# ericzzj1989/BALF

Measured on AMD Instinct MI355X. Metric: images/sec + keypoints/sec on 1080p gray (detector forward + NMS + top-K); NMS index match vs CPU ref, higher is better.
Workload: dtype f16 MFMA, split hi+lo operands (3 products), f32 accumulate/LN/GELU/softmax/NMS

## Files before the change

balf_amd/_lib.py:

```python
from __future__ import annotations

import ctypes as C
import os

_HERE = os.path.dirname(os.path.abspath(__file__))
LIB_PATH = os.environ.get("BALF_HIP_LIB", os.path.join(_HERE, "libbalf_hip.so"))

OK = 0
PREC_FP32, PREC_FP16 = 0, 1
MAX_NMS_SIZE, MAX_TOPK = 32, 16384
PYR_SRC_U8, PYR_SRC_F32, PYR_SRC_LEVEL = 0, 1, 2
PYR_MAX_RADIUS, MAX_PYRAMID_LEVELS = 8, 32
VAL_LEG_GREEDY, VAL_LEG_WINDOW = 0, 1
STATUS_SCORE, STATUS_RANGE, STATUS_SE, STATUS_WORDS = 0, 1, 2, 4

_vp, _i, _sz, _fp = C.c_void_p, C.c_int, C.c_size_t, C.c_void_p
PROTOTYPES = {
    "balf_abi_version": (_i, []),
    "balf_error_string": (C.c_char_p, [_i]),
    "balf_device_check": (_i, []),
    "balf_build_flags": (C.c_char_p, []),
    "balf_num_state_tensors": (_i, []),
    "balf_state_tensor_name": (C.c_char_p, [_i]),
    "balf_state_tensor_numel": (_sz, [_i]),
    "balf_packed_weights_bytes": (_sz, [_i]),
    "balf_pack_weights": (_i, [C.POINTER(_vp), _i, _i, _vp, _sz]),
    "balf_forward_workspace_bytes": (_sz, [_i, _i, _i]),
    "balf_forward_micro_batch": (_i, [_i, _i, _i]),
    "balf_forward": (_i, [_vp, _i, _fp, _i, _i, _i, _fp, _fp, _vp, _sz, _vp]),
    "balf_forward_u8": (_i, [_vp, _i, _vp, _i, _i, _i, _i, _fp, _fp, _vp, _sz, _vp]),
    "balf_forward_status": (_i, [_vp, _i, _fp, _i, _i, _i, _fp, _fp, _vp, _sz, _vp, _vp]),
    "balf_forward_u8_status": (_i, [_vp, _i, _vp, _i, _i, _i, _i, _fp, _fp, _vp, _sz, _vp, _vp]),
    "balf_forward_stage_view_numel": (_sz, [_i, _i, _i, _i]),
    "balf_forward_stage_view": (_i, [_i, _vp, _sz, _i, _i, _i, _i, _fp, _vp]),
    "balf_window_nms": (_i, [_fp, _i, _i, _i, _i, _i, _fp, _vp]),
    "balf_nms_topk_workspace_bytes": (_sz, [_i, _i, _i, _i]),
    "balf_nms_topk": (_i, [_fp, _i, _i, _i, _i, _i, _i, _i, _i, _i, _i, _vp, _fp, _vp, _vp, _sz, _vp]),
    "balf_nms_threshold": (_i, [_fp, _i, _i, _i, _i, _i, _i, _i, _i, _i, C.c_float, _i, _vp, _fp, _vp, _vp, _sz, _vp]),
    "balf_pyramid_level": (_i, [_vp, _i, _i, _i, _i, _i, C.c_double, _i, _i, _fp, _vp]),
    "balf_nms_topk_budget": (_i, [_fp, _i, _i, _i, _i, _i, _i, _i, _i, _i, _i, _i, _vp, _vp, _fp, _vp, _vp, _sz, _vp]),
    "balf_multiscale_merge": (_i, [_vp, _fp, _vp, _i, _i, _i, _vp, _vp, _i, _i, _vp, _vp, _vp]),
    "balf_greedy_nms_workspace_bytes": (_sz, [_i, _i, _i, _i]),
    "balf_greedy_nms": (_i, [_fp, _i, _i, _i, _i, _i, _i, _i, _i, C.c_float, _i, _i, _i, _vp, _fp, _fp, _vp, _vp, _vp,
                            _sz, _vp]),
    "balf_hardnet_num_state_tensors": (_i, []),
    "balf_hardnet_state_tensor_name": (C.c_char_p, [_i]),
    "balf_hardnet_state_tensor_numel": (_sz, [_i]),
    "balf_hardnet_packed_weights_bytes": (_sz, []),
    "balf_hardnet_pack_weights": (_i, [C.POINTER(_vp), _i, _vp, _sz]),
    "balf_hardnet_workspace_bytes": (_sz, [_i]),
    "balf_hardnet_forward": (_i, [_vp, _fp, _i, _fp, _vp, _sz, _vp]),
    "balf_hardnet_forward_masked": (_i, [_vp, _fp, _i, _i, _vp, _fp, _vp, _sz, _vp]),
    "balf_hardnet_forward_ex": (_i, [_vp, _fp, _i, _i, _vp, _i, _fp, _vp, _sz, _vp]),
    "balf_extract_patches_workspace_bytes": (_sz, [_i, _i, C.c_float]),
    "balf_extract_patches": (_i, [_vp, _i, _i, _fp, _i, C.c_float, _fp, _vp, _sz, _vp]),
    "balf_extract_patches_batch_workspace_bytes": (_sz, [_i, _i, _i, C.c_float]),
    "balf_extract_patches_batch": (_i, [_vp, _i, _i, _i, _fp, _vp, _i, C.c_float, _fp, _vp, _sz, _vp]),
    "balf_rgb_to_gray": (_i, [_vp, C.c_long, _vp, _vp]),
    "balf_match_smnn_workspace_bytes": (_sz, [_i, _i]),
    "balf_match_smnn": (_i, [_fp, _i, _fp, _i, C.c_float, _vp, _fp, _vp, _vp, _sz, _vp]),
    "balf_match_smnn_batch_workspace_bytes": (_sz, [_i, _i, _i]),
    "balf_match_smnn_batch": (_i, [_fp, _i, _vp, _fp, _i, _vp, _i, C.c_float, _vp, _fp, _vp, _vp, _sz, _vp]),
    "balf_repeatability_workspace_bytes": (_sz, [_i, _i, _i]),
    "balf_repeatability": (_i, [_vp, _i, _vp, _i, C.c_double, C.c_double, C.c_double, C.c_double, _i, _vp, _vp, _vp, _vp,
                               _vp, _sz, _vp]),
    "balf_apply_homography": (_i, [_vp, _i, _vp, _vp, _vp]),
    "balf_common_region_masks": (_i, [_vp, _i, _i, _i, _i, _i, _vp, _vp, _vp]),
    "balf_common_points_batch": (_i, [_vp, _vp, _i, _vp, _vp, _i, _i, _vp, _vp, _vp, _vp, _vp, _vp, _vp]),
    "balf_repeatability_batch_workspace_bytes": (_sz, [_i, _i, _i, _i]),
    "balf_repeatability_batch": (_i, [_vp, _vp, _i, _i, _vp, _vp, _i, _i, _i, _i, C.c_double, C.c_double, C.c_double,
                                     C.c_double, _i, _vp, _vp, _vp, _sz, _vp]),
    "balf_common_points_index_batch": (_i, [_vp, _vp, _i, _vp, _vp, _i, _i, _vp, _vp, _vp, _vp, _vp, _vp, _vp, _vp, _vp]),
    "balf_match_accuracy_batch": (_i, [_vp, _i, _vp, _i, _vp, _vp, _vp, _i, _i, C.POINTER(C.c_double), _i, _vp, _vp, _vp]),
    "balf_val_points_workspace_bytes": (_sz, [_i, _i, _i, _i, _i, _i, _i, _i]),
    "balf_val_points": (_i, [_fp, _i, _i, _fp, _i, _i, _i, _vp, _i, C.c_float, _i, _i, _vp, _vp, _vp, _vp, _sz, _vp]),
    "balf_resize_repeatability_batch_workspace_bytes": (_sz, [_i, _i, _i, _i]),
    "balf_resize_repeatability_batch": (_i, [_vp, _vp, _i, _i, _vp, _vp, _i, _i, _i, _i, _i, _vp, _vp, _vp, _i, C.c_double,
                                            _vp, _vp, _vp, _sz, _vp]),
    "balf_resize_crop_u8": (_i, [_vp, _sz, _vp, _vp, _i, _i, _i, _i, _vp, _vp]),
    "balf_synth_pairs_workspace_bytes": (_sz, [_i, _i]),
    "balf_synth_pairs": (_i, [_vp, _sz, _vp, _vp, _i, _vp, _vp, _vp, _fp, _i, _vp, _i, _i, _fp, _fp, _fp, _fp, _vp, _vp, _sz,
                             _vp]),
    "balf_detector_loss_workspace_bytes": (_sz, [_i, _i, _i]),
    "balf_detector_loss": (_i, [_fp, _fp, _fp, _fp, _i, _i, _i, _fp, _fp, _vp, _fp, _vp, _sz, _vp]),
    "balf_head_train_workspace_bytes": (_sz, [C.c_long]),
    "balf_head_train_saved_bytes": (_sz, [C.c_long]),
    "balf_head_train_forward": (_i, [_fp, _fp, _fp, _fp, _fp, _fp, _fp, _i, _i, _i, C.c_double, _i, _fp, _fp, _fp, _fp, _fp,
                                    C.c_double, _vp, _vp, _sz, _vp]),
    "balf_head_train_backward": (_i, [_fp, _fp, _fp, _fp, _fp, _vp, _i, _i, _i, _fp, _fp, _fp, _fp, _fp, _fp, _fp, _vp, _sz, _vp]),
    "balf_rcab_train_workspace_bytes": (_sz, [_i, _i, _i]),
    "balf_rcab_train_saved_bytes": (_sz, [_i, _i, _i]),
# ... 102 lines not shown
```

balf_amd/csrc/nms_topk.hip:

```cpp
#include <cstdint>
#include <cstdlib>
#include "block_ops.h"
#include "common.h"
#include "prof.h"

namespace {

constexpr int TH = 64;
constexpr int TW = 64;
constexpr int SEG = 16;
constexpr int NTHREADS = 256;

template <int SIZE, int N>
__device__ __forceinline__ void window_max_1d(const float (&v)[N + SIZE - 1], float (&o)[N]) {
    if constexpr (SIZE == 15) {
        constexpr int L = N + 14;
        float a[L - 1], b[L - 3], c[L - 7];
#pragma unroll
        for (int i = 0; i < L - 1; ++i) a[i] = fmaxf(v[i], v[i + 1]);
#pragma unroll
        for (int i = 0; i < L - 3; ++i) b[i] = fmaxf(a[i], a[i + 2]);
#pragma unroll
        for (int i = 0; i < L - 7; ++i) c[i] = fmaxf(b[i], b[i + 4]);
#pragma unroll
        for (int i = 0; i < N; ++i) o[i] = fmaxf(c[i], c[i + 7]);
    } else {
#pragma unroll
        for (int i = 0; i < N; ++i) {
            float m = v[i];
#pragma unroll
            for (int k = 1; k < SIZE; ++k) m = fmaxf(m, v[i + k]);
            o[i] = m;
        }
    }
}

struct NmsArgs {
    const float *src;
    int Hs, Ws;
    int crop_y, crop_x;
    int H, W;
    int border;
    int size;
    int2 *surv;
    int *surv_count;
    long cap;
    float *dense;
};

__device__ __forceinline__ float load_score(const NmsArgs &a, const float *img, int y, int x) {
    if (y < 0 || y >= a.H || x < 0 || x >= a.W) return -INFINITY;
    if (y < a.border || y >= a.H - a.border || x < a.border || x >= a.W - a.border) return 0.0f;
    return img[(long)(a.crop_y + y) * a.Ws + (a.crop_x + x)];
// ... 237 lines not shown
    const int b = blockIdx.z;
    const int ty0 = blockIdx.y * TH, tx0 = blockIdx.x * TW;
    const float *img = a.src + (long)b * a.Hs * a.Ws;
    const int tid = threadIdx.x;

    for (int i = tid; i < IN_H * IN_W; i += NTHREADS) {
        const int r = i / IN_W, c = i - r * IN_W;
        s_in[r * PIN + c] = load_score(a, img, ty0 - LO + r, tx0 - LO + c);
    }
    __syncthreads();
    for (int i = tid; i < IN_H * TW; i += NTHREADS) {
        const int r = i / TW, c = i - r * TW;
        float m = s_in[r * PIN + c];
        for (int k = 1; k < size; ++k) m = fmaxf(m, s_in[r * PIN + c + k]);
        s_row[r * PROW + c] = m;
    }
    __syncthreads();

    const int x = tid & (TW - 1), seg = tid / TW;
    const int gx = tx0 + x;
    unsigned keepmask = 0;
    float cen[SEG];
    for (int j = 0; j < SEG; ++j) {
        const int ry = seg * SEG + j;
        float m = s_row[ry * PROW + x];
        for (int k = 1; k < size; ++k) m = fmaxf(m, s_row[(ry + k) * PROW + x]);
        const int gy = ty0 + ry;
        cen[j] = s_in[(ry + LO) * PIN + x + LO];
        const bool inside = (gy < a.H) && (gx < a.W);
        const bool keep = inside && (cen[j] == m);
        if (a.dense != nullptr) {
            if (inside) a.dense[((long)b * a.H + gy) * a.W + gx] = cen[j] * (keep ? 1.0f : 0.0f);
        } else if (keep && cen[j] > 0.0f) {
            keepmask |= 1u << j;
        }
    }
    if (a.dense != nullptr) return;

    int total;
    const int excl = block_exclusive_scan(__popc(keepmask), s_scan, &total);
    if (total == 0) return;
    if (tid == 0) s_base = atomicAdd(&a.surv_count[b], total);
    __syncthreads();
    long pos = (long)b * a.cap + s_base + excl;
    for (int j = 0; j < SEG; ++j) {
        if (keepmask & (1u << j)) {
            const int gy = ty0 + seg * SEG + j;
            a.surv[pos++] = make_int2(gy * a.W + gx, __float_as_int(cen[j]));
        }
    }
}

constexpr int SEL_THREADS = 1024;

__global__ __launch_bounds__(SEL_THREADS) void topk_select_kernel(const int2 *surv_all, const int *surv_count,
                                                                  long cap, int K, int npow2, int zero_fallback,
                                                                  unsigned thr_explicit, int32_t *idx_out,
                                                                  float *score_out, int32_t *count_out,
                                                                  int32_t *taken, int cum_budget) {
    extern __shared__ __attribute__((aligned(16))) unsigned char smem[];
    unsigned long long *keys = reinterpret_cast<unsigned long long *>(smem);
    unsigned *s_hist = reinterpret_cast<unsigned *>(keys + npow2);
    int *s_tmp = reinterpret_cast<int *>(s_hist + 256);
    int *s_cnt = s_tmp + 4;

    const int b = blockIdx.x;
    const int2 *surv = surv_all + (long)b * cap;
    const int n = surv_count[b];
    const int K_row = K;
    int32_t *idx_o = idx_out + (long)b * K_row;
    float *sc_o = score_out + (long)b * K_row;
    if (taken) {
        if (threadIdx.x == 0) {
            long kb = (long)cum_budget - taken[b];
            kb = kb < cap ? kb : cap;
            kb = kb < K_row ? kb : K_row;
            *s_cnt = kb > 0 ? (int)kb : 0;
        }
        __syncthreads();
        K = *s_cnt;
        __syncthreads();
        npow2 = balf::next_pow2(K);
    }

    if (K == 0 || (n == 0 && (!zero_fallback || thr_explicit))) {
        for (int i = threadIdx.x; i < K_row; i += SEL_THREADS) { idx_o[i] = -1; sc_o[i] = 0.0f; }
        if (threadIdx.x == 0) count_out[b] = 0;
        return;
    }
    if (n == 0) {
        for (int i = threadIdx.x; i < K_row; i += SEL_THREADS) { idx_o[i] = i < K ? i : -1; sc_o[i] = 0.0f; }
        if (threadIdx.x == 0) {
            count_out[b] = K;
            if (taken) taken[b] += K;
        }
        return;
    }

    constexpr int CACHE = 16;
    const bool cached = n <= CACHE * SEL_THREADS;
    int2 ent[CACHE];
    if (cached) {
#pragma unroll
        for (int j = 0; j < CACHE; ++j) {
            const int i = threadIdx.x + j * SEL_THREADS;
            ent[j] = (i < n) ? surv[i] : make_int2(0x7fffffff, 0);
        }
    }
    const int n_mine = (n - (int)threadIdx.x + SEL_THREADS - 1) / SEL_THREADS;
    auto each = [&](auto f) {
        if (cached) {
#pragma unroll
            for (int j = 0; j < CACHE; ++j)
                if (j < n_mine) f(ent[j]);
        } else {
            for (int i = threadIdx.x; i < n; i += SEL_THREADS) f(surv[i]);
        }
    };

    unsigned thr = 0;
    int idx_cut = 0x7fffffff;
    auto raster_cut = [&]() {
        int d0, d1;
        const unsigned t = thr;
        return (int)balf::radix_select<32, false, SEL_THREADS>(
            K, [&](auto count) { each([&](int2 e) { if ((unsigned)e.y >= t) count((unsigned)e.x); }); }, s_hist, s_tmp, &d0, &d1);
    };
    if (thr_explicit) {
        thr = thr_explicit;
        if (threadIdx.x == 0) *s_cnt = 0;
        __syncthreads();
        int mine = 0;
        each([&](int2 e) { if ((unsigned)e.y >= thr) ++mine; });
        if (mine) atomicAdd(s_cnt, mine);
        __syncthreads();
        const int reach = *s_cnt;
        __syncthreads();
        if (reach > K) idx_cut = raster_cut();
    } else if (n > K) {
        int n_eq, need_eq;
        thr = (unsigned)balf::radix_select<32, true, SEL_THREADS>(
            K, [&](auto count) { each([&](int2 e) { count((unsigned)e.y); }); }, s_hist, s_tmp, &n_eq, &need_eq);
        if (n_eq > need_eq) idx_cut = raster_cut();
    }

    if (threadIdx.x == 0) *s_cnt = 0;
    for (int i = threadIdx.x; i < npow2; i += SEL_THREADS) keys[i] = ~0ull;
    __syncthreads();
    each([&](int2 e) {
        const unsigned sb = (unsigned)e.y;
        if (sb >= thr && e.x <= idx_cut) {
            const int p = atomicAdd(s_cnt, 1);
            keys[p] = ((unsigned long long)(~sb) << 32) | (unsigned)e.x;
        }
    });
    __syncthreads();
    const int cnt = *s_cnt;

    balf::bitonic_sort<SEL_THREADS>(keys, npow2);
    for (int i = threadIdx.x; i < K_row; i += SEL_THREADS) {
        if (i < cnt) {
            const unsigned long long kv = keys[i];
            idx_o[i] = (int32_t)(unsigned)(kv & 0xffffffffull);
            sc_o[i] = __uint_as_float(~(unsigned)(kv >> 32));
        } else {
            idx_o[i] = -1;
            sc_o[i] = 0.0f;
        }
    }
    if (threadIdx.x == 0) {
        count_out[b] = cnt;
        if (taken) taken[b] += cnt;
    }
}

int launch_nms_tiles(const NmsArgs &a, int B, hipStream_t stream) {
    dim3 grid(balf_ceil_div(a.W, TW), balf_ceil_div(a.H, TH), B), block(NTHREADS);
    if (balf_prof::g_on) balf_prof::before(balf_prof::kNmsTile, stream);
    static const bool no_vec = getenv("BALF_NMS_NO_VEC") != nullptr;
    if (a.size == 15 && a.dense == nullptr && !no_vec && a.Ws % 4 == 0 && a.crop_x % 4 == 0 &&
        (reinterpret_cast<uintptr_t>(a.src) & 15) == 0 && ((long)a.Hs * a.Ws) % 4 == 0) {
        hipLaunchKernelGGL(nms_tile15_vec_kernel, dim3(balf_ceil_div(a.W, TW), balf_ceil_div(a.H, V_TH), B), block, 0, stream, a);
        if (balf_prof::g_on) balf_prof::after(stream);
        BALF_LAUNCH_CHECK();
        return BALF_OK;
    }
    switch (a.size) {
        case 15: hipLaunchKernelGGL(nms_tile_kernel<15>, grid, block, 0, stream, a); break;
        case 5: hipLaunchKernelGGL(nms_tile_kernel<5>, grid, block, 0, stream, a); break;
        case 3: hipLaunchKernelGGL(nms_tile_kernel<3>, grid, block, 0, stream, a); break;
        default: hipLaunchKernelGGL(nms_tile_kernel_generic, grid, block, 0, stream, a); break;
    }
    if (balf_prof::g_on) balf_prof::after(stream);
    BALF_LAUNCH_CHECK();
    return BALF_OK;
}

}

namespace {
__global__ __launch_bounds__(256) void fill_u32_kernel(unsigned *dst, unsigned value, size_t n) {
    for (size_t i = (size_t)blockIdx.x * 256 + threadIdx.x; i < n; i += (size_t)gridDim.x * 256) dst[i] = value;
}
}

int balf_fill_u32(void *dst_dev, unsigned value, size_t n_words, hipStream_t stream) {
    if (n_words == 0) return BALF_OK;
    const size_t blocks = (n_words + 255) / 256;
    hipLaunchKernelGGL(fill_u32_kernel, dim3((unsigned)(blocks < 1024 ? blocks : 1024)), dim3(256), 0, stream,
                       static_cast<unsigned *>(dst_dev), value, n_words);
    BALF_LAUNCH_CHECK();
    return BALF_OK;
}

int balf_topk_select_launch(const int2 *surv, const int *counts, long cap, int B, int K, int zero_fallback,
                            int32_t *idx_dev, float *score_dev, int32_t *count_dev, hipStream_t st,
                            unsigned thr_explicit, int32_t *taken_dev, int cum_budget) {
    const int npow2 = balf::next_pow2(K);
    const size_t smem = (size_t)npow2 * 8 + 256 * 4 + 8 * 4;
    if (smem > 48 * 1024 &&
        hipFuncSetAttribute(reinterpret_cast<const void *>(topk_select_kernel),
                            hipFuncAttributeMaxDynamicSharedMemorySize, (int)smem) != hipSuccess)
        return BALF_ERR_LAUNCH;
    BALF_PROF(balf_prof::kTopkSelect, st,
              hipLaunchKernelGGL(topk_select_kernel, dim3(B), dim3(SEL_THREADS), smem, st, surv, counts, cap, K, npow2,
                                 zero_fallback, thr_explicit, idx_dev, score_dev, count_dev, taken_dev, cum_budget));
    BALF_LAUNCH_CHECK();
    return BALF_OK;
}

extern "C" int balf_window_nms(const float *score_dev, int B, int H, int W, int border, int nms_size,
                               float *out_dev, void *stream) {
    if (!score_dev || !out_dev || B <= 0 || H <= 0 || W <= 0 || border < 0) return BALF_ERR_ARG;
    if (nms_size < 1 || nms_size > BALF_MAX_NMS_SIZE) return BALF_ERR_ARG;
    if ((long)H * W > 0x7fffffffL) return BALF_ERR_SHAPE;
    NmsArgs a{score_dev, H, W, 0, 0, H, W, border, nms_size, nullptr, nullptr, 0, out_dev};
    return launch_nms_tiles(a, B, (hipStream_t)stream);
}

extern "C" size_t balf_nms_topk_workspace_bytes(int B, int H, int W, int K) {
    if (B <= 0 || H <= 0 || W <= 0 || K <= 0) return 0;
    return balf_align_up((size_t)B * sizeof(int), 256) + (size_t)B * (size_t)H * (size_t)W * sizeof(int2);
}

namespace {
int nms_select(const float *prob_dev, int B, int Hp, int Wp, int crop_y, int crop_x, int H, int W, int border,
               int nms_size, int K, unsigned thr_explicit, int32_t *idx_dev, float *score_dev, int32_t *count_dev,
               void *workspace_dev, size_t workspace_bytes, void *stream, int32_t *taken_dev = nullptr,
               int cum_budget = 0) {
    if (!prob_dev || !idx_dev || !score_dev || !count_dev || !workspace_dev) return BALF_ERR_ARG;
    if (B <= 0 || H <= 0 || W <= 0 || K <= 0 || border < 0) return BALF_ERR_ARG;
    if (nms_size < 1 || nms_size > BALF_MAX_NMS_SIZE || K > BALF_MAX_TOPK) return BALF_ERR_ARG;
    if (crop_y < 0 || crop_x < 0 || crop_y + H > Hp || crop_x + W > Wp) return BALF_ERR_SHAPE;
    if ((long)H * W > 0x7fffffffL || (!taken_dev && (long)K > (long)H * W)) return BALF_ERR_SHAPE;
    if (workspace_bytes < balf_nms_topk_workspace_bytes(B, H, W, K)) return BALF_ERR_WORKSPACE;
    hipStream_t st = (hipStream_t)stream;

    int *counts = reinterpret_cast<int *>(workspace_dev);
    int2 *surv = reinterpret_cast<int2 *>(reinterpret_cast<char *>(workspace_dev) +
                                          balf_align_up((size_t)B * sizeof(int), 256));
    if (balf_fill_u32(counts, 0u, balf_align_up((size_t)B * sizeof(int), 256) / 4, st) != BALF_OK) return BALF_ERR_LAUNCH;
    NmsArgs a{prob_dev, Hp, Wp, crop_y, crop_x, H, W, border, nms_size, surv, counts, (long)H * W, nullptr};
    int rc = launch_nms_tiles(a, B, st);
    if (rc != BALF_OK) return rc;

    return balf_topk_select_launch(surv, counts, (long)H * W, B, K, 1, idx_dev, score_dev, count_dev, st,
                                   thr_explicit, taken_dev, cum_budget);
}
}

int balf_window_survivors_launch(const float *prob_dev, int B, int H, int W, int nms_size, int2 *surv, int *counts,
                                 hipStream_t st) {
    if (balf_fill_u32(counts, 0u, (size_t)B, st) != BALF_OK) return BALF_ERR_LAUNCH;
    NmsArgs a{prob_dev, H, W, 0, 0, H, W, 0, nms_size, surv, counts, (long)H * W, nullptr};
    return launch_nms_tiles(a, B, st);
}

extern "C" int balf_nms_topk(const float *prob_dev, int B, int Hp, int Wp, int crop_y, int crop_x, int H, int W,
                             int border, int nms_size, int K, int32_t *idx_dev, float *score_dev,
                             int32_t *count_dev, void *workspace_dev, size_t workspace_bytes, void *stream) {
    return nms_select(prob_dev, B, Hp, Wp, crop_y, crop_x, H, W, border, nms_size, K, 0u, idx_dev, score_dev, count_dev,
                      workspace_dev, workspace_bytes, stream);
}

extern "C" int balf_nms_threshold(const float *prob_dev, int B, int Hp, int Wp, int crop_y, int crop_x, int H, int W,
                                  int border, int nms_size, float threshold, int K, int32_t *idx_dev, float *score_dev,
                                  int32_t *count_dev, void *workspace_dev, size_t workspace_bytes, void *stream) {
    if (!(threshold > 0.0f) || !(threshold < INFINITY)) return BALF_ERR_ARG;
    const unsigned bits = __builtin_bit_cast(unsigned, threshold);
    return nms_select(prob_dev, B, Hp, Wp, crop_y, crop_x, H, W, border, nms_size, K, bits, idx_dev, score_dev, count_dev,
                      workspace_dev, workspace_bytes, stream);
}

extern "C" int balf_nms_topk_budget(const float *prob_dev, int B, int Hp, int Wp, int crop_y, int crop_x, int H, int W,
                                    int border, int nms_size, int cum_budget, int K_max, int32_t *taken_dev,
                                    int32_t *idx_dev, float *score_dev, int32_t *count_dev, void *workspace_dev,
                                    size_t workspace_bytes, void *stream) {
    if (!taken_dev || cum_budget < 0 || cum_budget > K_max) return BALF_ERR_ARG;
    return nms_select(prob_dev, B, Hp, Wp, crop_y, crop_x, H, W, border, nms_size, K_max, 0u, idx_dev, score_dev, count_dev,
                      workspace_dev, workspace_bytes, stream, taken_dev, cum_budget);
}
```

balf_amd/ops.py:

```python
from __future__ import annotations

import ctypes as C
from typing import Dict, NamedTuple, Optional, Tuple

import numpy as np
import torch

from . import _lib
from .arch import padded_hw
from ._lib import BalfHipError, check, current_stream_ptr, lib, require_gpu_tensor

_workspaces: Dict[Tuple[str, int, int], torch.Tensor] = {}
_MAX_STREAMS_PER_TAG = 2


def _workspace(tag: str, device, nbytes: int) -> torch.Tensor:
    dev_index = device.index if device.index is not None else torch.cuda.current_device()
    key = (tag, dev_index, torch.cuda.current_stream(device).cuda_stream)
    ws = _workspaces.pop(key, None)
    if ws is None or ws.numel() < nbytes:
        ws = None
        with torch.cuda.device(device):
            ws = torch.empty(max(nbytes, 256), dtype=torch.uint8, device=device)
        same = [k for k in _workspaces if k[0] == tag and k[1] == dev_index]
        for k in same[:max(0, len(same) - (_MAX_STREAMS_PER_TAG - 1))]:
            del _workspaces[k]
    _workspaces[key] = ws
    return ws


def release_workspaces() -> None:
    _workspaces.clear()


def window_nms(score: torch.Tensor, border: int, nms_size: int) -> torch.Tensor:
    require_gpu_tensor(score, "score")
    if score.dtype != torch.float32 or score.dim() != 3:
        raise BalfHipError("score must be a [B,H,W] float32 tensor")
    out = torch.empty_like(score)
    b, h, w = score.shape
    with torch.cuda.device(score.device):
        check(lib().balf_window_nms(score.data_ptr(), b, h, w, int(border), int(nms_size), out.data_ptr(),
                                    current_stream_ptr(score.device)), "balf_window_nms")
    return out


def nms_topk(prob: torch.Tensor, crop_y: int, crop_x: int, h: int, w: int, border: int, nms_size: int,
             k: int, threshold: float = -1.0) -> Tuple[torch.Tensor, torch.Tensor, torch.Tensor]:
    require_gpu_tensor(prob, "prob")
    if prob.dtype != torch.float32 or prob.dim() != 3:
        raise BalfHipError("prob must be a [B,Hp,Wp] float32 tensor")
    if k > h * w:
        raise IndexError(f"index {k - 1} is out of bounds for axis 0 with size {h * w}")
    b, hp, wp = prob.shape
    dev = prob.device
    idx = torch.empty((b, k), dtype=torch.int32, device=dev)
    score = torch.empty((b, k), dtype=torch.float32, device=dev)
    count = torch.empty((b,), dtype=torch.int32, device=dev)
    nbytes = lib().balf_nms_topk_workspace_bytes(b, h, w, k)
    ws = _workspace("nms", dev, nbytes)
    with torch.cuda.device(dev):
        if threshold == -1:
            check(lib().balf_nms_topk(prob.data_ptr(), b, hp, wp, int(crop_y), int(crop_x), int(h), int(w),
                                      int(border), int(nms_size), int(k), idx.data_ptr(), score.data_ptr(),
                                      count.data_ptr(), ws.data_ptr(), ws.numel(), current_stream_ptr(dev)),
                  "balf_nms_topk")
        else:
            check(lib().balf_nms_threshold(prob.data_ptr(), b, hp, wp, int(crop_y), int(crop_x), int(h), int(w),
                                           int(border), int(nms_size), float(threshold), int(k), idx.data_ptr(),
                                           score.data_ptr(), count.data_ptr(), ws.data_ptr(), ws.numel(),
                                           current_stream_ptr(dev)), "balf_nms_threshold")
    return idx, score, count


def greedy_nms(prob: torch.Tensor, crop_y: int, crop_x: int, h: int, w: int, border: int, conf_thresh: float,
               dist_thresh: int, k: int, subpixel_patch: int = 0):
    require_gpu_tensor(prob, "prob")
    if prob.dtype != torch.float32 or prob.dim() != 3:
        raise BalfHipError("prob must be a [B,Hp,Wp] float32 tensor")
    b, hp, wp = prob.shape
    dev = prob.device
    idx = torch.empty((b, k), dtype=torch.int32, device=dev)
    score = torch.empty((b, k), dtype=torch.float32, device=dev)
    xy = torch.empty((b, k, 2), dtype=torch.float32, device=dev) if subpixel_patch > 0 else None
    count = torch.empty((b,), dtype=torch.int32, device=dev)
    total = torch.empty((b,), dtype=torch.int32, device=dev)
    ws = _workspace("greedy", dev, lib().balf_greedy_nms_workspace_bytes(b, h, w, k))
    with torch.cuda.device(dev):
        check(lib().balf_greedy_nms(prob.data_ptr(), b, hp, wp, int(crop_y), int(crop_x), int(h), int(w), int(border),
                                    float(conf_thresh), int(dist_thresh), int(k), int(subpixel_patch), idx.data_ptr(),
                                    score.data_ptr(), xy.data_ptr() if xy is not None else None, count.data_ptr(),
                                    total.data_ptr(), ws.data_ptr(), ws.numel(), current_stream_ptr(dev)),
              "balf_greedy_nms")
    return idx, score, xy, count, total


def profile_begin() -> None:
    check(lib().balf_profile_begin(), "balf_profile_begin")


def profile_end():
    l = lib()
    n = l.balf_profile_num_slots()
    ms = (C.c_float * n)()
    cnt = (C.c_int * n)()
    check(l.balf_profile_end(ms, cnt), "balf_profile_end")
    return {l.balf_profile_slot_name(i).decode(): (float(ms[i]), int(cnt[i])) for i in range(n) if cnt[i]}


def extract_patches(gray_u8: torch.Tensor, xy: torch.Tensor, scale: float) -> torch.Tensor:
    require_gpu_tensor(gray_u8, "gray_u8")
    if not xy.is_cuda:
        raise BalfHipError("xy must live on the GPU")
    if gray_u8.dtype != torch.uint8 or gray_u8.dim() != 2:
        raise BalfHipError("gray_u8 must be a [H,W] uint8 tensor")
    if xy.dim() != 2 or xy.shape[1] != 2:
        raise BalfHipError("xy must be [N,2]")
    xy = xy.contiguous().float()
    n = xy.shape[0]
    h, w = gray_u8.shape
    dev = gray_u8.device
    out = torch.empty((n, 1, 32, 32), dtype=torch.float32, device=dev)
    if n == 0:
        return out
    nbytes = lib().balf_extract_patches_workspace_bytes(h, w, float(scale))
# ... 729 lines not shown
```

balf_amd/pipeline.py:

```python
from __future__ import annotations

from typing import Optional, Tuple

import numpy as np
import torch

from . import arch, ops
from .guard import run_guarded
from .utils import test_utils as T


def detect_batch(model, x_pad: torch.Tensor, h: int, w: int, border: int = 15, nms_size: int = 15,
                 num_points: int = 1000, precomputed_offsets: Optional[Tuple[int, int]] = None, want_logits: bool = False):
    hp, wp = x_pad.shape[-2:]
    if precomputed_offsets is None:
        ehp, ewp, top, left = arch.padded_hw(h, w)
        if (ehp, ewp) != (hp, wp):
            raise ValueError(f"a {h}x{w} image pads to {ehp}x{ewp}, got {hp}x{wp}")
    else:
        top, left = precomputed_offsets
    prob = model(x_pad, want_logits=want_logits)["prob"]
    idx, score, count = ops.nms_topk(prob, top, left, h, w, border, nms_size, num_points)
    return idx, score, count, prob

# ... 62 lines not shown

@torch.no_grad()
def extract_detections(image_RGB_norm, model, device, cell_size=8, nms_size=15, num_points=25, border_size=15):
    h, w = image_RGB_norm.shape[0], image_RGB_norm.shape[1]
    x = pad_image_on_device(image_RGB_norm, device)

    def run():
        idx, score, count, prob = detect_batch(model, x, h, w, border_size, nms_size, num_points)
        return idx, score, int(count[0]), prob
    idx, score, n, prob = run_guarded(model, run)
    i = idx[0, :n].cpu().numpy().astype(np.int64)
    pts = np.empty((n, 4), dtype=np.float64)
    pts[:, 0], pts[:, 1], pts[:, 2], pts[:, 3] = i % w, i // w, 1.0, score[0, :n].cpu().numpy()
    _, _, top, left = arch.padded_hw(h, w)
    return pts, prob[:, top:top + h, left:left + w].unsqueeze(1)


def shard_range(total: int, rank: int, world: int) -> Tuple[int, int]:
    base, extra = divmod(total, world)
    lo = rank * base + min(rank, extra)
    return lo, lo + base + (1 if rank < extra else 0)


_SHAPES_CHECKED = set()


def allgather_keypoints(idx: torch.Tensor, score: torch.Tensor, count: torch.Tensor, group=None, force: bool = False,
                        total: Optional[int] = None):
    import torch.distributed as dist
    if not (dist.is_available() and dist.is_initialized()):
        return idx, score, count
    if dist.get_world_size(group) == 1 and not force:
        return idx, score, count
    world, rank = dist.get_world_size(group), dist.get_rank(group)
    b, k = idx.shape
    if total is None:
        rows = b
        key = (id(group) if group is not None else 0, world, b, k, str(idx.device))
        if key not in _SHAPES_CHECKED:
            mine = torch.tensor([b, k], dtype=torch.int64, device=idx.device)
            seen = torch.empty(world * 2, dtype=torch.int64, device=idx.device)
            dist.all_gather_into_tensor(seen, mine, group=group)
            seen = seen.view(world, 2)
            if not bool((seen == mine).all()):
                raise ValueError(f"allgather_keypoints: slab shapes differ across ranks ({seen.tolist()}); pass total= for the "
                                 f"unequal shards of shard_range")
            _SHAPES_CHECKED.add(key)
        shard_rows = [b] * world
    else:
        rows = -(-total // world)
        shard_rows = [shard_range(total, r, world)[1] - shard_range(total, r, world)[0] for r in range(world)]
        if shard_rows[rank] != b:
            raise ValueError(f"allgather_keypoints: rank {rank} of {world} holds {b} images, shard_range({total}) gives {shard_rows[rank]}")
    slab = torch.empty((rows, 2 * k + 1), dtype=torch.int32, device=idx.device)
    slab[:b, :k] = idx
    slab[:b, k:2 * k] = score.view(torch.int32)
    slab[:b, 2 * k] = count
    if rows > b:
        slab[b:, :k] = -1
        slab[b:, k:] = 0
    out = torch.empty((world * rows, 2 * k + 1), dtype=torch.int32, device=idx.device)
    dist.all_gather_into_tensor(out, slab, group=group)
    if any(r != rows for r in shard_rows):
        keep = torch.cat([torch.arange(r * rows, r * rows + shard_rows[r], device=idx.device) for r in range(world)])
        out = out.index_select(0, keep)
    return out[:, :k].contiguous(), out[:, k:2 * k].contiguous().view(torch.float32), out[:, 2 * k].contiguous()
```

include/balf_hip.h:

```cpp
#ifndef BALF_HIP_H
#define BALF_HIP_H

#include <stddef.h>
#include <stdint.h>

#ifdef __cplusplus
extern "C" {
#endif

#define BALF_ABI_VERSION 1

#define BALF_OK 0
#define BALF_ERR_ARG (-1)
#define BALF_ERR_SHAPE (-2)
#define BALF_ERR_WORKSPACE (-3)
#define BALF_ERR_ARCH (-4)
#define BALF_ERR_LAUNCH (-5)

#define BALF_MAX_NMS_SIZE 32
#define BALF_MAX_TOPK 16384

#define BALF_PREC_FP32 0
#define BALF_PREC_FP16 1

int balf_abi_version(void);
const char *balf_error_string(int code);
int balf_device_check(void);
const char *balf_build_flags(void);

int balf_num_state_tensors(void);
const char *balf_state_tensor_name(int i);
size_t balf_state_tensor_numel(int i);
size_t balf_packed_weights_bytes(int precision);
int balf_pack_weights(const float *const *tensors, int n_tensors, int precision,
                      void *packed_host, size_t packed_bytes);

size_t balf_forward_workspace_bytes(int B, int Hp, int Wp);
int balf_forward_micro_batch(int B, int Hp, int Wp);
int balf_forward(const void *packed_dev, int precision, const float *x_nchw_dev, int B, int Hp, int Wp,
                 float *logits_dev, float *prob_dev, void *workspace_dev, size_t workspace_bytes,
                 void *stream);

int balf_forward_u8(const void *packed_dev, int precision, const unsigned char *image_dev, int channels, int B,
                    int H, int W, float *logits_dev, float *prob_dev, void *workspace_dev, size_t workspace_bytes,
                    void *stream);

#define BALF_STATUS_SCORE 0
#define BALF_STATUS_RANGE 1
#define BALF_STATUS_SE 2
#define BALF_STATUS_WORDS 4
int balf_forward_status(const void *packed_dev, int precision, const float *x_nchw_dev, int B, int Hp, int Wp,
                        float *logits_dev, float *prob_dev, void *workspace_dev, size_t workspace_bytes,
                        int *status_dev, void *stream);
int balf_forward_u8_status(const void *packed_dev, int precision, const unsigned char *image_dev, int channels, int B,
                           int H, int W, float *logits_dev, float *prob_dev, void *workspace_dev, size_t workspace_bytes,
                           int *status_dev, void *stream);

size_t balf_forward_stage_view_numel(int B, int Hp, int Wp, int stage);
int balf_forward_stage_view(int precision, const void *workspace_dev, size_t workspace_bytes, int B, int Hp, int Wp, int stage,
                            float *out_dev, void *stream);

int balf_window_nms(const float *score_dev, int B, int H, int W, int border, int nms_size,
                    float *out_dev, void *stream);

size_t balf_nms_topk_workspace_bytes(int B, int H, int W, int K);
int balf_nms_topk(const float *prob_dev, int B, int Hp, int Wp, int crop_y, int crop_x, int H, int W,
                  int border, int nms_size, int K, int32_t *idx_dev, float *score_dev,
                  int32_t *count_dev, void *workspace_dev, size_t workspace_bytes, void *stream);

int balf_nms_threshold(const float *prob_dev, int B, int Hp, int Wp, int crop_y, int crop_x, int H, int W,
                       int border, int nms_size, float threshold, int K, int32_t *idx_dev, float *score_dev,
                       int32_t *count_dev, void *workspace_dev, size_t workspace_bytes, void *stream);

#define BALF_PYR_SRC_U8 0
#define BALF_PYR_SRC_F32 1
#define BALF_PYR_SRC_LEVEL 2
#define BALF_PYR_MAX_RADIUS 8
#define BALF_MAX_PYRAMID_LEVELS 32
int balf_pyramid_level(const void *src_dev, int src_kind, int channels, int B, int H_in, int W_in, double sigma, int H_out,
                       int W_out, float *dst_dev, void *stream);

int balf_nms_topk_budget(const float *prob_dev, int B, int Hp, int Wp, int crop_y, int crop_x, int H, int W, int border,
                         int nms_size, int cum_budget, int K_max, int32_t *taken_dev, int32_t *idx_dev, float *score_dev,
                         int32_t *count_dev, void *workspace_dev, size_t workspace_bytes, void *stream);

int balf_multiscale_merge(const int32_t *idx_dev, const float *score_dev, const int32_t *count_dev, int L, int B, int K_max,
                          const int32_t *level_w_host, const double *h_host, int N, int order_yx, double *pts_dev,
                          int32_t *count_out_dev, void *stream);

size_t balf_greedy_nms_workspace_bytes(int B, int H, int W, int K);
int balf_greedy_nms(const float *prob_dev, int B, int Hp, int Wp, int crop_y, int crop_x, int H, int W, int border,
                    float conf_thresh, int dist_thresh, int K, int subpixel_patch, int32_t *idx_dev,
                    float *score_dev, float *xy_dev, int32_t *count_dev, int32_t *total_dev, void *workspace_dev,
                    size_t workspace_bytes, void *stream);

int balf_hardnet_num_state_tensors(void);
const char *balf_hardnet_state_tensor_name(int i);
size_t balf_hardnet_state_tensor_numel(int i);
size_t balf_hardnet_packed_weights_bytes(void);
int balf_hardnet_pack_weights(const float *const *tensors, int n_tensors, void *packed_host, size_t packed_bytes);
size_t balf_hardnet_workspace_bytes(int n_patches);
int balf_hardnet_forward(const void *packed_dev, const float *patches_dev, int n_patches, float *desc_dev,
                         void *workspace_dev, size_t workspace_bytes, void *stream);
int balf_hardnet_forward_masked(const void *packed_dev, const float *patches_dev, int n_patches, int group,
                                const int32_t *count_dev, float *desc_dev, void *workspace_dev, size_t workspace_bytes,
                                void *stream);
#define BALF_HARDNET_SPLIT_F16 0
#define BALF_HARDNET_PLAIN_F16 1
int balf_hardnet_forward_ex(const void *packed_dev, const float *patches_dev, int n_patches, int group,
                            const int32_t *count_dev, int precision, float *desc_dev, void *workspace_dev,
                            size_t workspace_bytes, void *stream);

size_t balf_extract_patches_workspace_bytes(int H, int W, float scale);
int balf_extract_patches(const unsigned char *gray_dev, int H, int W, const float *xy_dev, int n_points, float scale,
                         float *patches_dev, void *workspace_dev, size_t workspace_bytes, void *stream);
size_t balf_extract_patches_batch_workspace_bytes(int B, int H, int W, float scale);
int balf_extract_patches_batch(const unsigned char *gray_dev, int B, int H, int W, const float *xy_dev,
                               const int32_t *count_dev, int K, float scale, float *patches_dev, void *workspace_dev,
                               size_t workspace_bytes, void *stream);
int balf_rgb_to_gray(const unsigned char *rgb_dev, long n_pixels, unsigned char *gray_dev, void *stream);
size_t balf_match_smnn_workspace_bytes(int n1, int n2);
size_t balf_match_smnn_batch_workspace_bytes(int pairs, int k1, int k2);
int balf_match_smnn_batch(const float *desc1_dev, int k1, const int32_t *n1_dev, const float *desc2_dev, int k2,
                          const int32_t *n2_dev, int pairs, float th, int32_t *idx_dev, float *dist_dev,
                          int32_t *count_dev, void *workspace_dev, size_t workspace_bytes, void *stream);
// ... 112 lines not shown
```

Baseline: 913.9.

## Split top-K select across CUs with global histogram, wave-level sort and output slab

Top-K selection now launches several blocks per image. Each block builds a 12-bit score histogram over a slice of the survivors and accumulates it into a global histogram, and the last block to arrive picks the threshold bin and runs a narrower radix select inside that bin. It also adds ballot-based compaction of the selected keys, a bitonic sort that does its small strides with wave shuffles, and a packed idx/score/count slab output so that all-gather can skip a repack copy. The aim is to use more CUs than images and to cut sort and compaction overhead, at the cost of extra workspace, global atomics and a last-block-done pattern that relies on relaxed ordering.

New measurement: 914.1, median of 6. About the same (+0.0%).

```diff
diff --git a/balf_amd/_lib.py b/balf_amd/_lib.py
--- a/balf_amd/_lib.py
+++ b/balf_amd/_lib.py
@@ -37,6 +37,7 @@
     "balf_nms_topk_workspace_bytes": (_sz, [_i, _i, _i, _i]),
     "balf_nms_topk": (_i, [_fp, _i, _i, _i, _i, _i, _i, _i, _i, _i, _i, _vp, _fp, _vp, _vp, _sz, _vp]),
     "balf_nms_threshold": (_i, [_fp, _i, _i, _i, _i, _i, _i, _i, _i, _i, C.c_float, _i, _vp, _fp, _vp, _vp, _sz, _vp]),
+    "balf_nms_topk_slab": (_i, [_fp, _i, _i, _i, _i, _i, _i, _i, _i, _i, C.c_float, _i, _vp, _vp, _sz, _vp]),
     "balf_pyramid_level": (_i, [_vp, _i, _i, _i, _i, _i, C.c_double, _i, _i, _fp, _vp]),
     "balf_nms_topk_budget": (_i, [_fp, _i, _i, _i, _i, _i, _i, _i, _i, _i, _i, _i, _vp, _vp, _fp, _vp, _vp, _sz, _vp]),
     "balf_multiscale_merge": (_i, [_vp, _fp, _vp, _i, _i, _i, _vp, _vp, _i, _i, _vp, _vp, _vp]),
diff --git a/balf_amd/csrc/nms_topk.hip b/balf_amd/csrc/nms_topk.hip
--- a/balf_amd/csrc/nms_topk.hip
+++ b/balf_amd/csrc/nms_topk.hip
@@ -1,4 +1,5 @@
 #include <cstdint>
+#include <atomic>
 #include <cstdlib>
 #include "block_ops.h"
 #include "common.h"
@@ -342,24 +343,88 @@
 }
 
 constexpr int SEL_THREADS = 1024;
+constexpr int SLICE_BITS = 12, SLICE_BINS = 1 << SLICE_BITS, SLICE_SHIFT = 31 - SLICE_BITS;
+constexpr int MAX_SLICES = 16;
+__device__ __forceinline__ unsigned slice_bin(unsigned score_bits) { return (score_bits >> SLICE_SHIFT) & (unsigned)(SLICE_BINS - 1); }
+
+__device__ __forceinline__ void bitonic_sort_in_waves(unsigned long long *keys, int n_pow2) {
+    if (n_pow2 < 64) {
+        balf::bitonic_sort<SEL_THREADS>(keys, n_pow2);
+        return;
+    }
+    auto exchange = [](unsigned long long x, int i, int j, int k) {
+        const unsigned long long y = __shfl_xor(x, j);
+        const bool keep_min = ((i & j) == 0) == ((i & k) == 0);
+        return keep_min ? (x < y ? x : y) : (x > y ? x : y);
+    };
+    for (int i = threadIdx.x; i < n_pow2; i += SEL_THREADS) {
+        unsigned long long x = keys[i];
+        for (int k = 2; k <= 64; k <<= 1)
+            for (int j = k >> 1; j > 0; j >>= 1) x = exchange(x, i, j, k);
+        keys[i] = x;
+    }
+    __syncthreads();
+    for (int k = 128; k <= n_pow2; k <<= 1) {
+        for (int j = k >> 1; j >= 64; j >>= 1) {
+            for (int i = threadIdx.x; i < n_pow2; i += SEL_THREADS) {
+                const int l = i ^ j;
+                if (l > i) {
+                    const unsigned long long x = keys[i], y = keys[l];
+                    if ((x > y) == ((i & k) == 0)) { keys[i] = y; keys[l] = x; }
+                }
+            }
+            __syncthreads();
+        }
+        for (int i = threadIdx.x; i < n_pow2; i += SEL_THREADS) {
+            unsigned long long x = keys[i];
+            for (int j = 32; j > 0; j >>= 1) x = exchange(x, i, j, k);
+            keys[i] = x;
+        }
+        __syncthreads();
+    }
+}
 
 __global__ __launch_bounds__(SEL_THREADS) void topk_select_kernel(const int2 *surv_all, const int *surv_count,
                                                                   long cap, int K, int npow2, int zero_fallback,
                                                                   unsigned thr_explicit, int32_t *idx_out,
                                                                   float *score_out, int32_t *count_out,
-                                                                  int32_t *taken, int cum_budget) {
+                                                                  int32_t *taken, int cum_budget, long row_stride,
+                                                                  long count_stride, int W, unsigned *g_hist, int *arrive) {
     extern __shared__ __attribute__((aligned(16))) unsigned char smem[];
     unsigned long long *keys = reinterpret_cast<unsigned long long *>(smem);
-    unsigned *s_hist = reinterpret_cast<unsigned *>(keys + npow2);
+    const int key_slots = (W > 1 && npow2 < SLICE_BINS / 2) ? SLICE_BINS / 2 : npow2;
+    unsigned *s_hist = reinterpret_cast<unsigned *>(keys + key_slots);
     int *s_tmp = reinterpret_cast<int *>(s_hist + 256);
     int *s_cnt = s_tmp + 4;
 
-    const int b = blockIdx.x;
+    const int b = blockIdx.x / W;
     const int2 *surv = surv_all + (long)b * cap;
     const int n = surv_count[b];
+    if (W > 1) {
+        unsigned *s_h = reinterpret_cast<unsigned *>(smem);
+        const int s = blockIdx.x - b * W;
+        for (int i = threadIdx.x; i < SLICE_BINS; i += SEL_THREADS) s_h[i] = 0;
+        __syncthreads();
+        for (long i = (long)s * SEL_THREADS + threadIdx.x; i < n; i += (long)W * SEL_THREADS)
+            atomicAdd(&s_h[slice_bin((unsigned)surv[i].y)], 1u);
+        __syncthreads();
+        unsigned seen = 0;
+        for (int i = threadIdx.x; i < SLICE_BINS; i += SEL_THREADS) {
+            const unsigned c = s_h[i];
+            if (c) seen += __hip_atomic_fetch_add(&g_hist[(long)b * SLICE_BINS + i], c, __ATOMIC_RELAXED, __HIP_MEMORY_SCOPE_AGENT);
+        }
+        asm volatile("" ::"v"(seen));
+        __syncthreads();
+        if (threadIdx.x == 0) *s_cnt = (__hip_atomic_fetch_add(&arrive[b], 1, __ATOMIC_RELAXED, __HIP_MEMORY_SCOPE_AGENT) == W - 1);
+        __syncthreads();
+        const bool last = *s_cnt != 0;
+        __syncthreads();
+        if (!last) return;
+    }
     const int K_row = K;
-    int32_t *idx_o = idx_out + (long)b * K_row;
-    float *sc_o = score_out + (long)b * K_row;
+    int32_t *idx_o = idx_out + (long)b * row_stride;
+    float *sc_o = score_out + (long)b * row_stride;
+    int32_t *cnt_o = count_out + (long)b * count_stride;
     if (taken) {
         if (threadIdx.x == 0) {
             long kb = (long)cum_budget - taken[b];
@@ -375,13 +440,13 @@
 
     if (K == 0 || (n == 0 && (!zero_fallback || thr_explicit))) {
         for (int i = threadIdx.x; i < K_row; i += SEL_THREADS) { idx_o[i] = -1; sc_o[i] = 0.0f; }
-        if (threadIdx.x == 0) count_out[b] = 0;
+        if (threadIdx.x == 0) *cnt_o = 0;
         return;
     }
     if (n == 0) {
         for (int i = threadIdx.x; i < K_row; i += SEL_THREADS) { idx_o[i] = i < K ? i : -1; sc_o[i] = 0.0f; }
         if (threadIdx.x == 0) {
-            count_out[b] = K;
+            *cnt_o = K;
             if (taken) taken[b] += K;
         }
         return;
@@ -429,25 +494,80 @@
         if (reach > K) idx_cut = raster_cut();
     } else if (n > K) {
         int n_eq, need_eq;
-        thr = (unsigned)balf::radix_select<32, true, SEL_THREADS>(
-            K, [&](auto count) { each([&](int2 e) { count((unsigned)e.y); }); }, s_hist, s_tmp, &n_eq, &need_eq);
+        if (W > 1) {
+            static_assert(SLICE_BINS == 4 * SEL_THREADS, "four bins per thread");
+            const unsigned *gh = g_hist + (long)b * SLICE_BINS;
+            int h[4], sum = 0;
+#pragma unroll
+            for (int i = 0; i < 4; ++i) {
+                h[i] = (int)__hip_atomic_load(gh + (SLICE_BINS - 1 - (4 * (int)threadIdx.x + i)), __ATOMIC_RELAXED, __HIP_MEMORY_SCOPE_AGENT);
+                sum += h[i];
+            }
+            const int lane = threadIdx.x & 63, wave = threadIdx.x >> 6;
+            const int winc = balf::wave_incl_scan(sum);
+            int *s_w = reinterpret_cast<int *>(s_hist);
+            if (lane == 63) s_w[wave] = winc;
+            __syncthreads();
+            int cum = winc - sum;
+            for (int w = 0; w < wave; ++w) cum += s_w[w];
+            if (cum < K && K <= cum + sum) {
+#pragma unroll
+                for (int i = 0; i < 4; ++i) {
+                    if (cum + h[i] >= K) {
+                        s_tmp[0] = SLICE_BINS - 1 - (4 * (int)threadIdx.x + i);
+                        s_tmp[1] = K - cum;
+                        break;
+                    }
+                    cum += h[i];
+                }
+            }
+            __syncthreads();
+            const unsigned bin = (unsigned)s_tmp[0];
+            const int rank = s_tmp[1];
+            __syncthreads();
+            constexpr unsigned LOW = (1u << SLICE_SHIFT) - 1u;
+            const unsigned low = (unsigned)balf::radix_select<24, true, SEL_THREADS>(
+                rank, [&](auto count) { each([&](int2 e) { if (slice_bin((unsigned)e.y) == bin) count((unsigned)e.y & LOW); }); },
+                s_hist, s_tmp, &n_eq, &need_eq);
+            thr = (bin << SLICE_SHIFT) | low;
+        } else {
+            thr = (unsigned)balf::radix_select<32, true, SEL_THREADS>(
+                K, [&](auto count) { each([&](int2 e) { count((unsigned)e.y); }); }, s_hist, s_tmp, &n_eq, &need_eq);
+        }
         if (n_eq > need_eq) idx_cut = raster_cut();
     }
 
     if (threadIdx.x == 0) *s_cnt = 0;
     for (int i = threadIdx.x; i < npow2; i += SEL_THREADS) keys[i] = ~0ull;
     __syncthreads();
-    each([&](int2 e) {
-        const unsigned sb = (unsigned)e.y;
-        if (sb >= thr && e.x <= idx_cut) {
-            const int p = atomicAdd(s_cnt, 1);
-            keys[p] = ((unsigned long long)(~sb) << 32) | (unsigned)e.x;
-        }
-    });
+    if (cached) {
+        const int lane = threadIdx.x & 63;
+#pragma unroll
+        for (int j = 0; j < CACHE; ++j) {
+            const unsigned sb = (unsigned)ent[j].y;
+            const bool sel = j < n_mine && sb >= thr && ent[j].x <= idx_cut;
+            const unsigned long long m = __ballot(sel);
+            if (m) {
+                const int first = __builtin_ctzll(m);
+                int base = 0;
+                if (lane == first) base = atomicAdd(s_cnt, __popcll(m));
+                base = __shfl(base, first);
+                if (sel) keys[base + __popcll(m & ((1ull << lane) - 1ull))] = ((unsigned long long)(~sb) << 32) | (unsigned)ent[j].x;
+            }
+        }
+    } else {
+        each([&](int2 e) {
+            const unsigned sb = (unsigned)e.y;
+            if (sb >= thr && e.x <= idx_cut) {
+                const int p = atomicAdd(s_cnt, 1);
+                keys[p] = ((unsigned long long)(~sb) << 32) | (unsigned)e.x;
+            }
+        });
+    }
     __syncthreads();
     const int cnt = *s_cnt;
 
-    balf::bitonic_sort<SEL_THREADS>(keys, npow2);
+    bitonic_sort_in_waves(keys, npow2);
     for (int i = threadIdx.x; i < K_row; i += SEL_THREADS) {
         if (i < cnt) {
             const unsigned long long kv = keys[i];
@@ -459,7 +579,7 @@
         }
     }
     if (threadIdx.x == 0) {
-        count_out[b] = cnt;
+        *cnt_o = cnt;
         if (taken) taken[b] += cnt;
     }
 }
@@ -489,6 +609,8 @@
 }
 
 namespace {
+size_t nms_header_bytes(int B) { return balf_align_up((size_t)2 * B * sizeof(int), 256); }
+
 __global__ __launch_bounds__(256) void fill_u32_kernel(unsigned *dst, unsigned value, size_t n) {
     for (size_t i = (size_t)blockIdx.x * 256 + threadIdx.x; i < n; i += (size_t)gridDim.x * 256) dst[i] = value;
 }
@@ -503,18 +625,34 @@
     return BALF_OK;
 }
 
+int balf_topk_select_launch_strided(const int2 *surv, const int *counts, long cap, int B, int K, int zero_fallback,
+                                    int32_t *idx_dev, float *score_dev, int32_t *count_dev, hipStream_t st,
+                                    unsigned thr_explicit, int32_t *taken_dev, int cum_budget, long row_stride,
+                                    long count_stride, int slices = 1, unsigned *hist_dev = nullptr, int *arrive_dev = nullptr);
+
 int balf_topk_select_launch(const int2 *surv, const int *counts, long cap, int B, int K, int zero_fallback,
                             int32_t *idx_dev, float *score_dev, int32_t *count_dev, hipStream_t st,
                             unsigned thr_explicit, int32_t *taken_dev, int cum_budget) {
+    return balf_topk_select_launch_strided(surv, counts, cap, B, K, zero_fallback, idx_dev, score_dev, count_dev, st, thr_explicit,
+                                           taken_dev, cum_budget, K, 1);
+}
+
+int balf_topk_select_launch_strided(const int2 *surv, const int *counts, long cap, int B, int K, int zero_fallback,
+                                    int32_t *idx_dev, float *score_dev, int32_t *count_dev, hipStream_t st,
+                                    unsigned thr_explicit, int32_t *taken_dev, int cum_budget, long row_stride,
+                                    long count_stride, int slices, unsigned *hist_dev, int *arrive_dev) {
+    if (slices < 1 || slices > MAX_SLICES || (slices > 1 && (!hist_dev || !arrive_dev))) return BALF_ERR_ARG;
     const int npow2 = balf::next_pow2(K);
-    const size_t smem = (size_t)npow2 * 8 + 256 * 4 + 8 * 4;
+    const size_t key_slots = (slices > 1 && npow2 < SLICE_BINS / 2) ? SLICE_BINS / 2 : npow2;
+    const size_t smem = key_slots * 8 + 256 * 4 + 8 * 4;
     if (smem > 48 * 1024 &&
         hipFuncSetAttribute(reinterpret_cast<const void *>(topk_select_kernel),
                             hipFuncAttributeMaxDynamicSharedMemorySize, (int)smem) != hipSuccess)
         return BALF_ERR_LAUNCH;
     BALF_PROF(balf_prof::kTopkSelect, st,
-              hipLaunchKernelGGL(topk_select_kernel, dim3(B), dim3(SEL_THREADS), smem, st, surv, counts, cap, K, npow2,
-                                 zero_fallback, thr_explicit, idx_dev, score_dev, count_dev, taken_dev, cum_budget));
+              hipLaunchKernelGGL(topk_select_kernel, dim3((unsigned)B * slices), dim3(SEL_THREADS), smem, st, surv, counts, cap, K, npow2,
+                                 zero_fallback, thr_explicit, idx_dev, score_dev, count_dev, taken_dev, cum_budget, row_stride,
+                                 count_stride, slices, hist_dev, arrive_dev));
     BALF_LAUNCH_CHECK();
     return BALF_OK;
 }
@@ -530,14 +668,29 @@
 
 extern "C" size_t balf_nms_topk_workspace_bytes(int B, int H, int W, int K) {
     if (B <= 0 || H <= 0 || W <= 0 || K <= 0) return 0;
-    return balf_align_up((size_t)B * sizeof(int), 256) + (size_t)B * (size_t)H * (size_t)W * sizeof(int2);
+    return nms_header_bytes(B) + (size_t)B * SLICE_BINS * sizeof(unsigned) + (size_t)B * (size_t)H * (size_t)W * sizeof(int2);
+}
+
+namespace {
+int topk_slices(int B) {
+    static std::atomic<int> cus[64];
+    int dev = 0;
+    if (hipGetDevice(&dev) != hipSuccess || dev < 0 || dev >= 64) return 1;
+    int n = cus[dev].load(std::memory_order_relaxed);
+    if (n == 0) {
+        if (hipDeviceGetAttribute(&n, hipDeviceAttributeMultiprocessorCount, dev) != hipSuccess || n <= 0) return 1;
+        cus[dev].store(n, std::memory_order_relaxed);
+    }
+    const int w = n / B;
+    return w < 1 ? 1 : (w > MAX_SLICES ? MAX_SLICES : w);
+}
 }
 
 namespace {
 int nms_select(const float *prob_dev, int B, int Hp, int Wp, int crop_y, int crop_x, int H, int W, int border,
                int nms_size, int K, unsigned thr_explicit, int32_t *idx_dev, float *score_dev, int32_t *count_dev,
                void *workspace_dev, size_t workspace_bytes, void *stream, int32_t *taken_dev = nullptr,
-               int cum_budget = 0) {
+               int cum_budget = 0, long row_stride = 0, long count_stride = 1) {
     if (!prob_dev || !idx_dev || !score_dev || !count_dev || !workspace_dev) return BALF_ERR_ARG;
     if (B <= 0 || H <= 0 || W <= 0 || K <= 0 || border < 0) return BALF_ERR_ARG;
     if (nms_size < 1 || nms_size > BALF_MAX_NMS_SIZE || K > BALF_MAX_TOPK) return BALF_ERR_ARG;
@@ -546,16 +699,19 @@
     if (workspace_bytes < balf_nms_topk_workspace_bytes(B, H, W, K)) return BALF_ERR_WORKSPACE;
     hipStream_t st = (hipStream_t)stream;
 
-    int *counts = reinterpret_cast<int *>(workspace_dev);
-    int2 *surv = reinterpret_cast<int2 *>(reinterpret_cast<char *>(workspace_dev) +
-                                          balf_align_up((size_t)B * sizeof(int), 256));
-    if (balf_fill_u32(counts, 0u, balf_align_up((size_t)B * sizeof(int), 256) / 4, st) != BALF_OK) return BALF_ERR_LAUNCH;
+    const int slices = thr_explicit ? 1 : topk_slices(B);
+    const size_t hdr = nms_header_bytes(B), hist_bytes = (size_t)B * SLICE_BINS * sizeof(unsigned);
+    int *counts = reinterpret_cast<int *>(workspace_dev), *arrive = counts + B;
+    unsigned *hist = reinterpret_cast<unsigned *>(reinterpret_cast<char *>(workspace_dev) + hdr);
+    int2 *surv = reinterpret_cast<int2 *>(reinterpret_cast<char *>(workspace_dev) + hdr + hist_bytes);
+    if (balf_fill_u32(counts, 0u, (hdr + (slices > 1 ? hist_bytes : 0)) / 4, st) != BALF_OK) return BALF_ERR_LAUNCH;
     NmsArgs a{prob_dev, Hp, Wp, crop_y, crop_x, H, W, border, nms_size, surv, counts, (long)H * W, nullptr};
     int rc = launch_nms_tiles(a, B, st);
     if (rc != BALF_OK) return rc;
 
-    return balf_topk_select_launch(surv, counts, (long)H * W, B, K, 1, idx_dev, score_dev, count_dev, st,
-                                   thr_explicit, taken_dev, cum_budget);
+    return balf_topk_select_launch_strided(surv, counts, (long)H * W, B, K, 1, idx_dev, score_dev, count_dev, st,
+                                           thr_explicit, taken_dev, cum_budget, row_stride ? row_stride : K, count_stride, slices, hist,
+                                           arrive);
 }
 }
 
@@ -590,3 +746,18 @@
     return nms_select(prob_dev, B, Hp, Wp, crop_y, crop_x, H, W, border, nms_size, K_max, 0u, idx_dev, score_dev, count_dev,
                       workspace_dev, workspace_bytes, stream, taken_dev, cum_budget);
 }
+
+extern "C" int balf_nms_topk_slab(const float *prob_dev, int B, int Hp, int Wp, int crop_y, int crop_x, int H, int W,
+                                  int border, int nms_size, float threshold, int K, int32_t *slab_dev, void *workspace_dev,
+                                  size_t workspace_bytes, void *stream) {
+    unsigned bits = 0u;
+    if (threshold != -1.0f) {
+        if (!(threshold > 0.0f) || !(threshold < INFINITY)) return BALF_ERR_ARG;
+        bits = __builtin_bit_cast(unsigned, threshold);
+    }
+    if (!slab_dev || K <= 0) return BALF_ERR_ARG;
+    const long stride = 2L * K + 1;
+    return nms_select(prob_dev, B, Hp, Wp, crop_y, crop_x, H, W, border, nms_size, K, bits, slab_dev,
+                      reinterpret_cast<float *>(slab_dev + K), slab_dev + 2L * K, workspace_dev, workspace_bytes, stream, nullptr, 0,
+                      stride, stride);
+}
diff --git a/balf_amd/ops.py b/balf_amd/ops.py
--- a/balf_amd/ops.py
+++ b/balf_amd/ops.py
@@ -54,23 +54,44 @@
         raise IndexError(f"index {k - 1} is out of bounds for axis 0 with size {h * w}")
     b, hp, wp = prob.shape
     dev = prob.device
-    idx = torch.empty((b, k), dtype=torch.int32, device=dev)
-    score = torch.empty((b, k), dtype=torch.float32, device=dev)
-    count = torch.empty((b,), dtype=torch.int32, device=dev)
+    slab = torch.empty((b, 2 * k + 1), dtype=torch.int32, device=dev)
     nbytes = lib().balf_nms_topk_workspace_bytes(b, h, w, k)
     ws = _workspace("nms", dev, nbytes)
     with torch.cuda.device(dev):
-        if threshold == -1:
-            check(lib().balf_nms_topk(prob.data_ptr(), b, hp, wp, int(crop_y), int(crop_x), int(h), int(w),
-                                      int(border), int(nms_size), int(k), idx.data_ptr(), score.data_ptr(),
-                                      count.data_ptr(), ws.data_ptr(), ws.numel(), current_stream_ptr(dev)),
-                  "balf_nms_topk")
-        else:
-            check(lib().balf_nms_threshold(prob.data_ptr(), b, hp, wp, int(crop_y), int(crop_x), int(h), int(w),
-                                           int(border), int(nms_size), float(threshold), int(k), idx.data_ptr(),
-                                           score.data_ptr(), count.data_ptr(), ws.data_ptr(), ws.numel(),
-                                           current_stream_ptr(dev)), "balf_nms_threshold")
-    return idx, score, count
+        check(lib().balf_nms_topk_slab(prob.data_ptr(), b, hp, wp, int(crop_y), int(crop_x), int(h), int(w),
+                                       int(border), int(nms_size), -1.0 if threshold == -1 else float(threshold), int(k),
+                                       slab.data_ptr(), ws.data_ptr(), ws.numel(), current_stream_ptr(dev)),
+              "balf_nms_topk_slab")
+    return keypoint_slab_views(slab)
+
+
+def keypoint_slab_views(slab: torch.Tensor) -> Tuple[torch.Tensor, torch.Tensor, torch.Tensor]:
+    k = (slab.shape[1] - 1) // 2
+    return slab[:, :k], slab[:, k:2 * k].view(torch.float32), slab[:, 2 * k]
+
+
+def keypoint_slab_of(idx: torch.Tensor, score: torch.Tensor, count: torch.Tensor) -> Optional[torch.Tensor]:
+    if idx.dim() != 2 or score.shape != idx.shape or count.dim() != 1 or count.shape[0] != idx.shape[0]:
+        return None
+    if idx.dtype != torch.int32 or score.dtype != torch.float32 or count.dtype != torch.int32:
+        return None
+    if idx.device != score.device or idx.device != count.device:
+        return None
+    b, k = idx.shape
+    if b == 0 or k == 0:
+        return None
+    row = 2 * k + 1
+    o = idx.storage_offset()
+    if score.storage_offset() != o + k or count.storage_offset() != o + 2 * k:
+        return None
+    if idx.stride() != (row, 1) or score.stride() != (row, 1) or count.stride() != (row,):
+        return None
+    ptr = idx.untyped_storage().data_ptr()
+    if score.untyped_storage().data_ptr() != ptr or count.untyped_storage().data_ptr() != ptr:
+        return None
+    if idx.untyped_storage().nbytes() < (o + b * row) * 4:
+        return None
+    return idx.as_strided((b, row), (row, 1), o)
 
 
 def greedy_nms(prob: torch.Tensor, crop_y: int, crop_x: int, h: int, w: int, border: int, conf_thresh: float,
diff --git a/balf_amd/pipeline.py b/balf_amd/pipeline.py
--- a/balf_amd/pipeline.py
+++ b/balf_amd/pipeline.py
@@ -138,6 +138,21 @@
         shard_rows = [shard_range(total, r, world)[1] - shard_range(total, r, world)[0] for r in range(world)]
         if shard_rows[rank] != b:
             raise ValueError(f"allgather_keypoints: rank {rank} of {world} holds {b} images, shard_range({total}) gives {shard_rows[rank]}")
+    own = ops.keypoint_slab_of(idx, score, count)
+    if own is not None:
+        if rows > b:
+            slab = torch.empty((rows, 2 * k + 1), dtype=torch.int32, device=idx.device)
+            slab[:b] = own
+            slab[b:, :k] = -1
+            slab[b:, k:] = 0
+        else:
+            slab = own
+        out = torch.empty((world * rows, 2 * k + 1), dtype=torch.int32, device=idx.device)
+        dist.all_gather_into_tensor(out, slab, group=group)
+        if any(r != rows for r in shard_rows):
+            keep = torch.cat([torch.arange(r * rows, r * rows + shard_rows[r], device=idx.device) for r in range(world)])
+            out = out.index_select(0, keep)
+        return ops.keypoint_slab_views(out)
     slab = torch.empty((rows, 2 * k + 1), dtype=torch.int32, device=idx.device)
     slab[:b, :k] = idx
     slab[:b, k:2 * k] = score.view(torch.int32)
diff --git a/include/balf_hip.h b/include/balf_hip.h
--- a/include/balf_hip.h
+++ b/include/balf_hip.h
@@ -71,6 +71,10 @@
 int balf_nms_threshold(const float *prob_dev, int B, int Hp, int Wp, int crop_y, int crop_x, int H, int W,
                        int border, int nms_size, float threshold, int K, int32_t *idx_dev, float *score_dev,
                        int32_t *count_dev, void *workspace_dev, size_t workspace_bytes, void *stream);
+
+int balf_nms_topk_slab(const float *prob_dev, int B, int Hp, int Wp, int crop_y, int crop_x, int H, int W, int border,
+                       int nms_size, float threshold, int K, int32_t *slab_dev, void *workspace_dev,
+                       size_t workspace_bytes, void *stream);
 
 #define BALF_PYR_SRC_U8 0
 #define BALF_PYR_SRC_F32 1
```
